# ZucksLiu/OCTCubeM

Measured on AMD Instinct MI355X. Metric: 3D-MAE pretrain volumes/s (ViT-L, 60x256x256, mask 0.75), higher is better.
Workload: dtype bf16; 1 GPU; OCTCube ViT-L 3D-MAE pre-train step (fwd+bwd+all-reduce+AdamW), synthetic (1,60,256,256) volumes, mask_ratio 0.75, decoder 512x8x16; global_batch=256, micro_batch_per_gpu=128, accum_steps=2, parallelism=dp1

## Files before the change

### octcubem_amd/csrc/attn_bwd1w.hip

```cpp
#include "attn_bwd1w.hpp"
#include "attn_bwd_tail1.hpp"
#ifndef BWD1W_TAIL_DEPTH
#define BWD1W_TAIL_DEPTH 4
#endif
#include "../../include/octmae.h"

namespace octmae {

namespace bwd1w {

constexpr int HD = 32, NW = 4, KW = 128, NG = 4, KB = NW * KW;
constexpr int LA = 3;
constexpr int NB = LA + 1;
constexpr int NOLD = 3;
using T = Tile<HD>;
constexpr int QR = 0;
constexpr int OR_ = QR + NB * T::BYTES;
constexpr int CR = OR_ + NB * T::BYTES;
constexpr int IMG = CR + NB * 512;
constexpr int IMG_BUF = KB * 64;
constexpr int OLD = IMG + 2 * IMG_BUF;
constexpr int LDS = OLD + NOLD * 2 * NW * 1024;
constexpr int STG = IMG;
static_assert(LDS <= 160 * 1024, "LDS budget");
static_assert((CR % 128) == 0 && (IMG % 128) == 0 && (OLD % 128) == 0, "XOR chunk selectors act on address bits 0..6");

using namespace bwd1w_util;

#ifdef BWD1W_STAMP
__device__ unsigned g_bwd1w_stamp[512 * 4 * 2 * 10];
#define STAMP(k) asm volatile("s_memtime %0" : "=s"(st_[k]))
#define STAMP_ACCUM(s)                                                                                           \
  do {                                                                                                           \
    asm volatile("s_waitcnt lgkmcnt(0)" : "+s"(st_[0]), "+s"(st_[1]), "+s"(st_[2]), "+s"(st_[3]), "+s"(st_[4]), \
                 "+s"(st_[5]), "+s"(st_[6]), "+s"(st_[7]), "+s"(st_[8]), "+s"(st_[9]));                          \
    _Pragma("unroll") for (int k_ = 0; k_ < 9; ++k_) acc_[s][k_] += (unsigned)st_[k_ + 1] - (unsigned)st_[k_];  \
    acc_[s][9] += (unsigned)st_[0] - last_;                                                                      \
    last_ = (unsigned)st_[9];                                                                                    \
  } while (0)
#else
#define STAMP(k)
#define STAMP_ACCUM(s)
#endif

}

__global__ __launch_bounds__(256, 1) void attn_bwd_fused1w_kernel(const bf16_t* __restrict__ qkv, const bf16_t* __restrict__ dout,
                                                                  const float* __restrict__ rowc, float* __restrict__ dq_ws,
                                                                  bf16_t* __restrict__ dqkv, int N, int NPAD, int H, int nkb,
                                                                  float scale, int tail_key) {
  using namespace bwd1w;
  extern __shared__ __attribute__((aligned(128))) char smem[];
  const unsigned lds0 = (unsigned)(size_t)(__attribute__((address_space(3))) char*)smem;

  const int tid = threadIdx.x, lane = tid & 63;
  const int wid = __builtin_amdgcn_readfirstlane(tid >> 6);
  const int r = lane & 31, h = lane >> 5;
  const int bh = xcd_remap((int)blockIdx.x, (int)gridDim.x);
  const int b = bh / H, head = bh % H;
  const size_t rs = (size_t)3 * H * HD, os = (size_t)H * HD;
  const bf16_t* qb = qkv + (size_t)b * N * rs + (size_t)head * HD;
  const bf16_t* kb_ = qb + (size_t)H * HD;
  const bf16_t* vb_ = qb + (size_t)2 * H * HD;
  const bf16_t* dob = dout + (size_t)b * N * os + (size_t)head * HD;
  const float sc2 = scale * LOG2E;
  const bool half_drain = ((N - 1) & 63) < 32;
  const int ntiles = (N + 63) / 64;

  const bool isq = wid < 2;
  const i32x4_t rsD = isq ? make_rsrc(qb, (unsigned)(((size_t)(N - 1) * rs + HD) * 2)) : make_rsrc(dob, (unsigned)(((size_t)(N - 1) * os + HD) * 2));
  unsigned dvoff[2], dlds[2];
#pragma unroll
  for (int i = 0; i < 2; ++i) {
    const int piece = (wid & 1) * 2 + i;
    const int q = piece * 64 + lane;
    const int row = q / T::CHUNKS, c = (q % T::CHUNKS) ^ T::sw(row);
    dvoff[i] = (unsigned)(((size_t)row * (isq ? rs : os) + c * 8) * 2);
    dlds[i] = (unsigned)((isq ? QR : OR_) + piece * 1024);
  }
  const unsigned dstride = (unsigned)(64 * (isq ? rs : os) * 2);
  const i32x4_t rsC = make_rsrc(rowc + (size_t)(wid & 1) * gridDim.x * NPAD + (size_t)bh * NPAD, (unsigned)((size_t)NPAD * 4));
  auto issue = [&](int dt, int ct, int slot) {
#pragma unroll
    for (int i = 0; i < 2; ++i) {
      const unsigned m0v = (unsigned)__builtin_amdgcn_readfirstlane((int)(lds0 + dlds[i] + (unsigned)(slot * T::BYTES)));
      lds_dma16(m0v, dvoff[i] + (unsigned)dt * dstride, rsD);
    }
    const unsigned m0c = (unsigned)__builtin_amdgcn_readfirstlane((int)(lds0 + CR + slot * 512 + (wid & 1) * 256));
    lds_dma4(m0c, (unsigned)((ct * 64 + lane) * 4), rsC);
  };

  float* wsb = dq_ws + (size_t)bh * N * HD;
  const i32x4_t rsW = make_rsrc(wsb, (unsigned)((size_t)N * HD * 4));
  const __amdgpu_buffer_rsrc_t rsWs = __builtin_amdgcn_make_buffer_rsrc(
      reinterpret_cast<void*>(((unsigned long long)(unsigned)rsW[1] << 32) | (unsigned)rsW[0]), 0, rsW[2], 0x00020000);
  const int dt = wid & 1, qt = wid >> 1, g16 = lane >> 4, c16 = lane & 15;
  const unsigned wsoff = (unsigned)(((16 * qt + c16) * HD + 16 * dt + 4 * g16) * 4);
  constexpr unsigned WS_SUB = 32 * HD * 4, WS_TILE = 64 * HD * 4, DROP = 0x80000000u;
  auto oldreq = [&](int tile, int buf, unsigned base) {
#pragma unroll
    for (int u = 0; u < 2; ++u) {
      const unsigned m0o = (unsigned)__builtin_amdgcn_readfirstlane((int)(lds0 + OLD + ((buf * 2 + u) * NW + wid) * 1024));
      lds_dma16_ws(m0o, wsoff + base + (unsigned)tile * WS_TILE + (unsigned)u * WS_SUB, rsW);
    }
  };

  const int tq_ = (lane >> 2) & 3, tp_ = lane & 3, tgi = (lane >> 4) & 1;
  const unsigned a_const = opaque(lds0 + (unsigned)(CR + 16 * h));
  const unsigned a_row = opaque(lds0 + (unsigned)(QR + T::off(r, h)));
  const unsigned a_trlo = opaque(lds0 + (unsigned)(QR + T::off(4 * h + tq_, 2 * tgi + (tp_ >> 1)) + (tp_ & 1) * 8));
  const unsigned a_trhi = opaque(lds0 + (unsigned)(QR + T::off(4 * h + tq_ + 8, 2 * tgi + (tp_ >> 1)) + (tp_ & 1) * 8));
  const unsigned a_imgw = opaque(lds0 + (unsigned)(IMG + img_off(wid * KW + r, h)));
  const unsigned a_imglo = opaque(lds0 + (unsigned)(IMG + img_off(8 * g16 + tq_, 4 * qt + tp_)));
  const unsigned a_imghi = opaque(lds0 + (unsigned)(IMG + img_off(8 * g16 + tq_ + 4, 4 * qt + tp_)));
  const unsigned a_old = opaque(lds0 + (unsigned)(OLD + wid * 1024 + lane * 16));
  f32x16 zero16;
#pragma unroll
  for (int e = 0; e < 16; ++e) zero16[e] = 0.f;
  const f32x4 zero4 = {0.f, 0.f, 0.f, 0.f};

  for (int kb = 0; kb < nkb; ++kb) {
    const int key0 = kb * KB;
    const unsigned oldbase = kb > 0 ? 0u : DROP;
    issue(0, 0, 0);
    issue(1, 1, 1);
    issue(2, 2, 2);
    oldreq(0, 0, oldbase);
    {
#pragma unroll
      for (int i = 0; i < KB * 4 / 256; ++i) {
        const int c = tid + 256 * i;
        const int row = c >> 2, cc = c & 3;
        const u32x4 v = *reinterpret_cast<const u32x4*>(kb_ + (size_t)(key0 + row) * rs + 8 * cc);
        *reinterpret_cast<u32x2*>(smem + STG + img_off(row, 2 * cc)) = u32x2{v[0], v[1]};
        *reinterpret_cast<u32x2*>(smem + STG + img_off(row, 2 * cc + 1)) = u32x2{v[2], v[3]};
      }
    }
    bf16x8 kS[NG][2], vS[NG][2];
#pragma unroll
    for (int g = 0; g < NG; ++g) {
      const size_t krow = (size_t)(key0 + wid * KW + 32 * g + r) * rs;
#pragma unroll
      for (int s = 0; s < 2; ++s) {
        const u32x4 kv = *reinterpret_cast<const u32x4*>(kb_ + krow + 16 * s + 8 * h);
        const u32x4 vv = *reinterpret_cast<const u32x4*>(vb_ + krow + 16 * s + 8 * h);
        kS[g][s] = scale_frag(kv, sc2);
        vS[g][s] = __builtin_bit_cast(bf16x8, vv);
      }
    }
    f32x16 dk0 = zero16, dk1 = zero16, dk2 = zero16, dk3 = zero16, dv0 = zero16, dv1 = zero16, dv2 = zero16, dv3 = zero16;
    __syncthreads();
    bf16x8 kT[KB / 32];
#pragma unroll
    for (int ks = 0; ks < KB / 32; ++ks)
      kT[ks] = cat4(lds_tr_read(smem + STG + img_off(8 * g16 + tq_, 4 * dt + tp_) + ks * 2048),
                    lds_tr_read(smem + STG + img_off(8 * g16 + tq_ + 4, 4 * dt + tp_) + ks * 2048));
    __builtin_amdgcn_s_waitcnt(0xC07F);
    __syncthreads();

    wait_vm<0>();
    __builtin_amdgcn_s_barrier();

    f32x16 lse_a, dlt_a, lse_b = zero16, dlt_b = zero16, saA, dpA, saB, dpB;
    f32x4 dqA = zero4, dqB = zero4;
    bf16x8 qrowa0, qrowa1, orowa0, orowa1, qrowb0, qrowb1, orowb0, orowb1, qTa0, qTa1, oTa0, oTa1, qTb0, qTb1, oTb0, oTb1;
    u32x4 pf0 = {0u, 0u, 0u, 0u}, pf1 = pf0, dsf0 = pf0, dsf1 = pf0;
    {
#pragma unroll
      for (int G = 0; G < 4; ++G) {
        const f32x4 a = lds_ld<f32x4>(a_const + 32 * G);
        const f32x4 d = lds_ld<f32x4>(a_const + 256 + 32 * G);
#pragma unroll
        for (int e = 0; e < 4; ++e) { lse_a[4 * G + e] = a[e]; dlt_a[4 * G + e] = d[e]; }
      }
      qrowa0 = lds_ld<bf16x8>(a_row);
      orowa0 = lds_ld<bf16x8>(a_row + (OR_ - QR));
      qrowa1 = lds_ld<bf16x8>(a_row ^ 32u);
      orowa1 = lds_ld<bf16x8>((a_row ^ 32u) + (OR_ - QR));
      qTa0 = cat4(lds_tr_ld(a_trlo), lds_tr_ld(a_trhi));
      oTa0 = cat4(lds_tr_ld(a_trlo + (OR_ - QR)), lds_tr_ld(a_trhi + (OR_ - QR)));
      qTa1 = cat4(lds_tr_ld(a_trlo + 16 * 64), lds_tr_ld(a_trhi + 16 * 64));
      oTa1 = cat4(lds_tr_ld(a_trlo + 16 * 64 + (OR_ - QR)), lds_tr_ld(a_trhi + 16 * 64 + (OR_ - QR)));
      qTb0 = qTb1 = oTb0 = oTb1 = qrowb0 = qrowb1 = orowb0 = orowb1 = __builtin_bit_cast(bf16x8, pf0);
      saA = mfma32(qrowa0, kS[0][0], lse_a);
      dpA = mfma32(orowa0, vS[0][0], dlt_a);
      saA = mfma32(qrowa1, kS[0][1], saA);
      dpA = mfma32(orowa1, vS[0][1], dpA);
      saB = zero16; dpB = zero16;
    }

#ifdef BWD1W_STAMP
    unsigned long long st_[10];
    unsigned acc_[2][10] = {};
    unsigned last_ = 0;
    STAMP(9);
    asm volatile("s_waitcnt lgkmcnt(0)" : "+s"(st_[9]));
    last_ = (unsigned)st_[9];
#endif
#define BWD1W_TILE_SETUP                                                                                            \
  [[maybe_unused]] const int slot = t & (NB - 1), slotn = (t + 1) & (NB - 1);                                                        \
  [[maybe_unused]] const unsigned s_pc1 = (unsigned)(slot * 512 + 128), s_x1 = (unsigned)(slot * T::BYTES + 32 * T::ROWB);           \
  [[maybe_unused]] const unsigned s_pcn = (unsigned)(slotn * 512), s_xn = (unsigned)(slotn * T::BYTES);                              \
  [[maybe_unused]] const unsigned s_oldr = (unsigned)(((t + 2) % NOLD) * 2 * NW * 1024);                                             \
  [[maybe_unused]] const unsigned s_redoff0 = t > 0 ? (unsigned)(t - 1) * WS_TILE : DROP;                                            \
  [[maybe_unused]] const unsigned s_redoff1 = t > 0 ? (unsigned)(t - 1) * WS_TILE + WS_SUB : DROP;                                   \
  [[maybe_unused]] auto issue_tile = [&]() {                                                                                         \
    const int tn = t + LA;                                                                                          \
    issue(tn < ntiles ? tn : tn - ntiles, tn < ntiles ? tn : ntiles, tn & (NB - 1));                                \
    oldreq(t + 1, (t + 1) % NOLD, oldbase);                                                                         \
  };
    const unsigned o_imglo = a_imglo, o_imghi = a_imghi, o_old = a_old, o_wsoff = wsoff;
#define BWD1W_DRAIN_ADDRS \
  [[maybe_unused]] const unsigned a_imglo = opaque(o_imglo), a_imghi = opaque(o_imghi), a_old = opaque(o_old), wsoff = opaque(o_wsoff);
#ifndef BWD1W_VMWAIT_EXTRA
#define BWD1W_VMWAIT_EXTRA 1
#endif
#define BWD1W_WAIT(t_) do { if ((t_) > 1) wait_vm<7 + BWD1W_VMWAIT_EXTRA>(); else wait_vm<7>(); } while (0)
    const int nloop = half_drain ? ntiles - 1 : ntiles;
    for (int t = 0; t < nloop; ++t) {
      if (t > 0) BWD1W_WAIT(t);
      BWD1W_TILE_SETUP
#include "attn_bwd1w_body.inc"
    }
    if (half_drain) {
      {
        const int t = ntiles - 1;
        BWD1W_WAIT(t);
        BWD1W_TILE_SETUP
#define BWD1W_ONLY_SUBSTEP0
#include "attn_bwd1w_body.inc"
#undef BWD1W_ONLY_SUBSTEP0
      {
        BWD1W_DRAIN_ADDRS
#define BWD1W_DRAIN_SLIM1
#include "attn_bwd1w_drain.inc"
#undef BWD1W_DRAIN_SLIM1
      }
      }
      {
        const int t = ntiles;
        BWD1W_WAIT(t);
        BWD1W_TILE_SETUP
        BWD1W_DRAIN_ADDRS
#define BWD1W_DRAIN_TINY0
#include "attn_bwd1w_drain.inc"
#undef BWD1W_DRAIN_TINY0
      }
    } else {
      const int t = ntiles;
      BWD1W_WAIT(t);
      BWD1W_TILE_SETUP
      BWD1W_DRAIN_ADDRS
#define BWD1W_DRAIN_SLIM0
#include "attn_bwd1w_drain.inc"
#undef BWD1W_DRAIN_SLIM0
#define BWD1W_DRAIN_TINY1
#include "attn_bwd1w_drain.inc"
#undef BWD1W_DRAIN_TINY1
    }
#undef BWD1W_TILE_SETUP
#undef BWD1W_DRAIN_ADDRS
#ifdef BWD1W_STAMP
    if (kb == 1 && lane == 0 && blockIdx.x < 512)
      for (int s_ = 0; s_ < 2; ++s_)
        for (int k_ = 0; k_ < 10; ++k_) g_bwd1w_stamp[((blockIdx.x * 4 + wid) * 2 + s_) * 10 + k_] = acc_[s_][k_];
#endif
    asm volatile("s_nop 15\n\ts_nop 15" : "+a"(dk0), "+a"(dk1), "+a"(dk2), "+a"(dk3), "+a"(dv0), "+a"(dv1), "+a"(dv2), "+a"(dv3));
    {
      const f32x16* dks[4] = {&dk0, &dk1, &dk2, &dk3};
      const f32x16* dvs[4] = {&dv0, &dv1, &dv2, &dv3};
#pragma unroll
      for (int g = 0; g < NG; ++g) {
        bf16_t* drow = dqkv + ((size_t)b * N + key0 + wid * KW + 32 * g + r) * rs + (size_t)head * HD;
        const f32x16& dkg = *dks[g];
        const f32x16& dvg = *dvs[g];
#pragma unroll
        for (int G = 0; G < 4; ++G) {
          const u32x2 wk = {pack2bf(dkg[4 * G] * scale, dkg[4 * G + 1] * scale), pack2bf(dkg[4 * G + 2] * scale, dkg[4 * G + 3] * scale)};
          const u32x2 wv = {pack2bf(dvg[4 * G], dvg[4 * G + 1]), pack2bf(dvg[4 * G + 2], dvg[4 * G + 3])};
          *reinterpret_cast<u32x2*>(drow + (size_t)H * HD + 8 * G + 4 * h) = wk;
          *reinterpret_cast<u32x2*>(drow + (size_t)2 * H * HD + 8 * G + 4 * h) = wv;
        }
      }
    }
  }
  wait_vm<0>();
  if (tail_key >= 0) {
    __syncthreads();
    const int lane_t = lane_id_fresh();
    attn_bwd_tail1_body<HD, BWD1W_TAIL_DEPTH>(qkv, dout, rowc, dq_ws, dqkv, N, NPAD, H, tail_key, 1, scale, bh, (int)gridDim.x, reinterpret_cast<float*>(smem),
                               wid * 64 + lane_t);
  }
}

}

using namespace octmae;

#ifdef BWD1W_STAMP
extern "C" int octmae_debug_bwd1w_stamps(void* host, int nbytes) {
  return (int)hipMemcpyFromSymbol(host, HIP_SYMBOL(octmae::bwd1w::g_bwd1w_stamp), (size_t)nbytes);
}
#endif

namespace octmae {
int launch_attn_bwd_fused1w(const bf16_t* qkv, const bf16_t* dout, const float* rowc, float* dq_ws, bf16_t* dqkv, int B, int N, int NPAD,
                            int H, int nkb, float scale, int tail_key, hipStream_t st) {
  static DynLdsOnce once;
  if (int rc = once.ensure(reinterpret_cast<const void*>(attn_bwd_fused1w_kernel), bwd1w::LDS)) return rc;
  hipLaunchKernelGGL(attn_bwd_fused1w_kernel, dim3(B * H), dim3(256), bwd1w::LDS, st, qkv, dout, rowc, dq_ws, dqkv, N, NPAD, H, nkb, scale, tail_key);
  OCTMAE_LAUNCH_CHECK();
  return 0;
}
}
```

### octcubem_amd/csrc/attn_bwd1w.hpp

```cpp
#pragma once
#include "attn_tile.hpp"

namespace octmae {
namespace bwd1w_util {

typedef __attribute__((ext_vector_type(4))) float f32x4_t;
__device__ __forceinline__ f32x4 mfma16(bf16x8 a, bf16x8 b, f32x4 c) { return mfma16x16(a, b, c); }

template <int CNT>
__device__ __forceinline__ void wait_vm() {
  static_assert(CNT >= 0 && CNT < 64, "vmcnt is 6 bits");
  __builtin_amdgcn_s_waitcnt((CNT & 15) | ((CNT >> 4) << 14) | (7 << 4) | (15 << 8));
}
__device__ __forceinline__ void lds_dma16(unsigned m0v, unsigned voff, i32x4_t rsrc) {
  asm volatile("s_mov_b32 m0, %0\n\tbuffer_load_dwordx4 %1, %2, 0 offen lds" ::"s"(m0v), "v"(voff), "s"(rsrc) : "memory", "m0");
}
#ifndef BWD1W_WS_ST_AUX
#define BWD1W_WS_ST_AUX 0
#endif
#ifdef BWD1W_ST_SMALL
#define BWD1W_RVO(x) ((x) & 0xFFFFu)
#else
#define BWD1W_RVO(x) (x)
#endif
__device__ __forceinline__ void lds_dma16_ws(unsigned m0v, unsigned voff, i32x4_t rsrc) {
#ifdef BWD1W_WS_LD_NT
  asm volatile("s_mov_b32 m0, %0\n\tbuffer_load_dwordx4 %1, %2, 0 offen nt lds" ::"s"(m0v), "v"(voff), "s"(rsrc) : "memory", "m0");
#else
  asm volatile("s_mov_b32 m0, %0\n\tbuffer_load_dwordx4 %1, %2, 0 offen lds" ::"s"(m0v), "v"(voff), "s"(rsrc) : "memory", "m0");
#endif
}
__device__ __forceinline__ void lds_dma4(unsigned m0v, unsigned voff, i32x4_t rsrc) {
  asm volatile("s_mov_b32 m0, %0\n\tbuffer_load_dword %1, %2, 0 offen lds" ::"s"(m0v), "v"(voff), "s"(rsrc) : "memory", "m0");
}
__device__ __forceinline__ i32x4_t make_rsrc(const void* base, unsigned bytes) {
  const unsigned long long a = (unsigned long long)base;
  i32x4_t r = {(int)(unsigned)a, (int)(unsigned)(a >> 32), (int)bytes, 0x00020000};
  r[0] = __builtin_amdgcn_readfirstlane(r[0]);
  r[1] = __builtin_amdgcn_readfirstlane(r[1]);
  r[2] = __builtin_amdgcn_readfirstlane(r[2]);
  r[3] = __builtin_amdgcn_readfirstlane(r[3]);
  return r;
}
__device__ __forceinline__ int img_off(int row, int c8) { return row * 64 + ((c8 ^ ((row >> 1) & 7)) << 3); }

#define MFMA_ACC(acc, a, b) asm volatile(OCTMAE_MFMA32_ASM " %0, %1, %2, %0" : "+a"(acc) : "v"(a), "v"(b))
__device__ __forceinline__ int lane_id_fresh() {
  int x;
  asm volatile("v_mbcnt_lo_u32_b32 %0, -1, 0\n\tv_mbcnt_hi_u32_b32 %0, -1, %0" : "=v"(x));
  return x;
}
#ifdef ABL_NO_BARRIER
#define SUBSTEP_END(N) __builtin_amdgcn_s_waitcnt(0xC07F | 0)
#else
#define SUBSTEP_END(N)                                            \
  do {                                                            \
    __builtin_amdgcn_s_waitcnt(0xC07F | ((N) << 8));              \
    __builtin_amdgcn_s_barrier();                                 \
  } while (0)
#endif

}
}
```

### octcubem_amd/csrc/attn_bwd1w64.hip

```cpp
#include "attn_bwd1w.hpp"
#include "attn_bwd_tail1.hpp"
#ifndef BWD1W_TAIL_DEPTH
#define BWD1W_TAIL_DEPTH 4
#endif
#include "../../include/octmae.h"

namespace octmae {

namespace bwd1w64 {

constexpr int HD = 64, NW = 4, KW = 64, NG = 2, KB = NW * KW;
constexpr int LA = 3;
constexpr int NB = LA + 1;
constexpr int NOLD = 3;
using T = Tile<HD>;
constexpr int QR = 0;
constexpr int OR_ = QR + NB * T::BYTES;
constexpr int CR = OR_ + NB * T::BYTES;
constexpr int IMG = CR + NB * 512;
constexpr int IMG_BUF = KB * 64;
constexpr int OLD = IMG + 2 * IMG_BUF;
constexpr int OLD_TILE = 2 * 2 * NW * 1024;
constexpr int LDS = OLD + NOLD * OLD_TILE;
constexpr int STG = IMG;
static_assert(KB * HD * 2 <= 2 * IMG_BUF, "K staging must fit the two images");
static_assert(LDS <= 160 * 1024, "LDS budget");
static_assert((CR % 128) == 0 && (IMG % 128) == 0 && (OLD % 128) == 0, "XOR chunk selectors act on address bits 0..6");
static_assert((OR_ - QR) % 128 == 0 && T::BYTES % 128 == 0, "slot / region offsets leave the low 7 address bits alone");

using namespace bwd1w_util;

__device__ __forceinline__ int kst_off(int row, int c) {
  const int sw = (row & 1) | (((row >> 2) & 1) << 1) | (((row >> 1) & 1) << 2) | (((row >> 3) & 1) << 3);
  return row * 128 + ((c ^ sw) << 3);
}

#ifdef BWD1W_STAMP
__device__ unsigned g_bwd1w64_stamp[512 * 4 * 2 * 8];
#define STAMP(k) asm volatile("s_memtime %0" : "=s"(st_[k]))
#define STAMP_ACCUM(s)                                                                                                         \
  do {                                                                                                                         \
    asm volatile("s_waitcnt lgkmcnt(0)" : "+s"(st_[0]), "+s"(st_[1]), "+s"(st_[2]), "+s"(st_[3]), "+s"(st_[4]), "+s"(st_[5])); \
    _Pragma("unroll") for (int k_ = 0; k_ < 5; ++k_) acc_[s][k_] += (unsigned)st_[k_ + 1] - (unsigned)st_[k_];                \
    acc_[s][5] += (unsigned)st_[0] - last_;                                                                                    \
    last_ = (unsigned)st_[5];                                                                                                  \
  } while (0)
#else
#define STAMP(k)
#define STAMP_ACCUM(s)
#endif

}

__global__ __launch_bounds__(256, 1) void attn_bwd_fused1w64_kernel(const bf16_t* __restrict__ qkv, const bf16_t* __restrict__ dout,
                                                                    const float* __restrict__ rowc, float* __restrict__ dq_ws,
                                                                    bf16_t* __restrict__ dqkv, int N, int NPAD, int H, int nkb,
                                                                    float scale, int tail_key) {
  using namespace bwd1w64;
  extern __shared__ __attribute__((aligned(128))) char smem[];
  const unsigned lds0 = (unsigned)(size_t)(__attribute__((address_space(3))) char*)smem;

  const int tid = threadIdx.x, lane = tid & 63;
  const int wid = __builtin_amdgcn_readfirstlane(tid >> 6);
  const int r = lane & 31, h = lane >> 5;
  const int bh = xcd_remap((int)blockIdx.x, (int)gridDim.x);
  const int b = bh / H, head = bh % H;
  const size_t rs = (size_t)3 * H * HD, os = (size_t)H * HD;
  const bf16_t* qb = qkv + (size_t)b * N * rs + (size_t)head * HD;
  const bf16_t* kb_ = qb + (size_t)H * HD;
  const bf16_t* vb_ = qb + (size_t)2 * H * HD;
  const bf16_t* dob = dout + (size_t)b * N * os + (size_t)head * HD;
  const float sc2 = scale * LOG2E;
  const bool half_drain = ((N - 1) & 63) < 32;
  const int ntiles = (N + 63) / 64;

  const bool isq = wid < 2;
  const i32x4_t rsD = isq ? make_rsrc(qb, (unsigned)(((size_t)(N - 1) * rs + HD) * 2)) : make_rsrc(dob, (unsigned)(((size_t)(N - 1) * os + HD) * 2));
  unsigned dvoff[4], dlds[4];
#pragma unroll
  for (int i = 0; i < 4; ++i) {
    const int piece = (wid & 1) * 4 + i;
    const int q = piece * 64 + lane;
    const int row = q / T::CHUNKS, c = (q % T::CHUNKS) ^ T::sw(row);
    dvoff[i] = (unsigned)(((size_t)row * (isq ? rs : os) + c * 8) * 2);
    dlds[i] = (unsigned)((isq ? QR : OR_) + piece * 1024);
  }
  const unsigned dstride = (unsigned)(64 * (isq ? rs : os) * 2);
  const i32x4_t rsC = make_rsrc(rowc + (size_t)(wid & 1) * gridDim.x * NPAD + (size_t)bh * NPAD, (unsigned)((size_t)NPAD * 4));
  auto issue = [&](int dt, int ct, int slot) {
#pragma unroll
    for (int i = 0; i < 4; ++i) {
      const unsigned m0v = (unsigned)__builtin_amdgcn_readfirstlane((int)(lds0 + dlds[i] + (unsigned)(slot * T::BYTES)));
      lds_dma16(m0v, dvoff[i] + (unsigned)dt * dstride, rsD);
    }
    const unsigned m0c = (unsigned)__builtin_amdgcn_readfirstlane((int)(lds0 + CR + slot * 512 + (wid & 1) * 256));
    lds_dma4(m0c, (unsigned)((ct * 64 + lane) * 4), rsC);
  };

  float* wsb = dq_ws + (size_t)bh * N * HD;
  const i32x4_t rsW = make_rsrc(wsb, (unsigned)((size_t)N * HD * 4));
  const __amdgpu_buffer_rsrc_t rsWs = __builtin_amdgcn_make_buffer_rsrc(
      reinterpret_cast<void*>(((unsigned long long)(unsigned)rsW[1] << 32) | (unsigned)rsW[0]), 0, rsW[2], 0x00020000);
  const int g16 = lane >> 4, c16 = lane & 15;
#ifdef ABL_TILED_WS
  const unsigned wsoff = (unsigned)(wid * 1024 + lane * 16);
#else
  const unsigned wsoff = (unsigned)((c16 * HD + 16 * wid + 4 * g16) * 4);
#endif
  constexpr unsigned WS_QT = 16 * HD * 4, WS_SUB = 32 * HD * 4, WS_TILE = 64 * HD * 4, DROP = 0x80000000u;
  static_assert(WS_QT == 4096, "the generated body stores the second query tile at + 4096");
  auto oldreq = [&](int tile, int buf, unsigned base) {
#pragma unroll
    for (int u = 0; u < 4; ++u) {
      const unsigned m0o = (unsigned)__builtin_amdgcn_readfirstlane((int)(lds0 + OLD + buf * OLD_TILE + (u * NW + wid) * 1024));
      lds_dma16_ws(m0o, wsoff + base + (unsigned)tile * WS_TILE + (unsigned)(u >> 1) * WS_SUB + (unsigned)(u & 1) * WS_QT, rsW);
    }
  };

  const int tq_ = (lane >> 2) & 3, tp_ = lane & 3, tgi = (lane >> 4) & 1;
  const unsigned a_const = opaque(lds0 + (unsigned)(CR + 16 * h));
  const unsigned a_row = opaque(lds0 + (unsigned)(QR + T::off(r, h)));
  const unsigned a_trlo = opaque(lds0 + (unsigned)(QR + T::off(4 * h + tq_, 2 * tgi + (tp_ >> 1)) + (tp_ & 1) * 8));
  const unsigned a_trhi = opaque(lds0 + (unsigned)(QR + T::off(4 * h + tq_ + 8, 2 * tgi + (tp_ >> 1)) + (tp_ & 1) * 8));
  const unsigned a_imgw = opaque(lds0 + (unsigned)(IMG + img_off(wid * KW + r, h)));
  const unsigned a_imglo = opaque(lds0 + (unsigned)(IMG + img_off(8 * g16 + tq_, tp_)));
  const unsigned a_imghi = opaque(lds0 + (unsigned)(IMG + img_off(8 * g16 + tq_ + 4, tp_)));
  const unsigned a_old = opaque(lds0 + (unsigned)(OLD + wid * 1024 + lane * 16));
  f32x16 zero16;
#pragma unroll
  for (int e = 0; e < 16; ++e) zero16[e] = 0.f;
  const f32x4 zero4 = {0.f, 0.f, 0.f, 0.f};

#ifdef BWD1W_STAMP
  unsigned long long k0_, r0_;
  asm volatile("s_memtime %0\n\ts_memrealtime %1\n\ts_waitcnt lgkmcnt(0)" : "=s"(k0_), "=s"(r0_));
#endif
  for (int kb = 0; kb < nkb; ++kb) {
    const int key0 = kb * KB;
    const unsigned oldbase = kb > 0 ? 0u : DROP;
    issue(0, 0, 0);
    issue(1, 1, 1);
    issue(2, 2, 2);
    oldreq(0, 0, oldbase);
    {
#pragma unroll
      for (int i = 0; i < KB * 8 / 256; ++i) {
        const int c = tid + 256 * i;
        const int row = c >> 3, cc = c & 7;
        const u32x4 v = *reinterpret_cast<const u32x4*>(kb_ + (size_t)(key0 + row) * rs + 8 * cc);
        *reinterpret_cast<u32x2*>(smem + STG + kst_off(row, 2 * cc)) = u32x2{v[0], v[1]};
        *reinterpret_cast<u32x2*>(smem + STG + kst_off(row, 2 * cc + 1)) = u32x2{v[2], v[3]};
      }
    }
    bf16x8 kS[NG][4], vS[NG][4];
#pragma unroll
    for (int g = 0; g < NG; ++g) {
      const size_t krow = (size_t)(key0 + wid * KW + 32 * g + r) * rs;
#pragma unroll
      for (int s = 0; s < 4; ++s) {
        const u32x4 kv = *reinterpret_cast<const u32x4*>(kb_ + krow + 16 * s + 8 * h);
        const u32x4 vv = *reinterpret_cast<const u32x4*>(vb_ + krow + 16 * s + 8 * h);
        kS[g][s] = scale_frag(kv, sc2);
        vS[g][s] = __builtin_bit_cast(bf16x8, vv);
      }
    }
    f32x16 dk00 = zero16, dk01 = zero16, dk10 = zero16, dk11 = zero16, dv00 = zero16, dv01 = zero16, dv10 = zero16, dv11 = zero16;
    __syncthreads();
    bf16x8 kT[KB / 32];
#pragma unroll
    for (int ks = 0; ks < KB / 32; ++ks)
      kT[ks] = cat4(lds_tr_read(smem + STG + kst_off(8 * g16 + tq_, 4 * wid + tp_) + ks * 32 * 128),
                    lds_tr_read(smem + STG + kst_off(8 * g16 + tq_ + 4, 4 * wid + tp_) + ks * 32 * 128));
    __builtin_amdgcn_s_waitcnt(0xC07F);
    __syncthreads();

    wait_vm<0>();
    __builtin_amdgcn_s_barrier();

    f32x16 lse_t, dlt_t, saA, dpA, saB = zero16, dpB = zero16;
    f32x4 dqA0 = zero4, dqA1 = zero4, dqB0 = zero4, dqB1 = zero4;
    bf16x8 qrow0, qrow1, qrow2, qrow3, orow0, orow1, orow2, orow3, qT0d0, qT0d1, oT0d0, oT0d1, qT1d0, qT1d1, oT1d0, oT1d1;
    u32x4 pf0 = {0u, 0u, 0u, 0u}, pf1 = pf0, dsf0 = pf0, dsf1 = pf0;
    {
#pragma unroll
      for (int G = 0; G < 4; ++G) {
        const f32x4 a = lds_ld<f32x4>(a_const + 32 * G);
        const f32x4 d = lds_ld<f32x4>(a_const + 256 + 32 * G);
#pragma unroll
        for (int e = 0; e < 4; ++e) { lse_t[4 * G + e] = a[e]; dlt_t[4 * G + e] = d[e]; }
      }
      qrow0 = lds_ld<bf16x8>(a_row);
      orow0 = lds_ld<bf16x8>(a_row + (OR_ - QR));
      qrow1 = lds_ld<bf16x8>(a_row ^ 32u);
      orow1 = lds_ld<bf16x8>((a_row ^ 32u) + (OR_ - QR));
      qrow2 = lds_ld<bf16x8>(a_row ^ 64u);
      orow2 = lds_ld<bf16x8>((a_row ^ 64u) + (OR_ - QR));
      qrow3 = lds_ld<bf16x8>(a_row ^ 96u);
      orow3 = lds_ld<bf16x8>((a_row ^ 96u) + (OR_ - QR));
      qT0d0 = cat4(lds_tr_ld(a_trlo), lds_tr_ld(a_trhi));
      oT0d0 = cat4(lds_tr_ld(a_trlo + (OR_ - QR)), lds_tr_ld(a_trhi + (OR_ - QR)));
      qT0d1 = cat4(lds_tr_ld(a_trlo ^ 64u), lds_tr_ld(a_trhi ^ 64u));
      oT0d1 = cat4(lds_tr_ld((a_trlo ^ 64u) + (OR_ - QR)), lds_tr_ld((a_trhi ^ 64u) + (OR_ - QR)));
      qT1d0 = qT1d1 = oT1d0 = oT1d1 = __builtin_bit_cast(bf16x8, pf0);
      saA = mfma32(qrow0, kS[0][0], lse_t);
      dpA = mfma32(orow0, vS[0][0], dlt_t);
      saA = mfma32(qrow1, kS[0][1], saA);
      dpA = mfma32(orow1, vS[0][1], dpA);
      saA = mfma32(qrow2, kS[0][2], saA);
      dpA = mfma32(orow2, vS[0][2], dpA);
      saA = mfma32(qrow3, kS[0][3], saA);
      dpA = mfma32(orow3, vS[0][3], dpA);
    }

#ifdef BWD1W_STAMP
    unsigned long long st_[6], sw_[2];
    unsigned acc_[2][8] = {};
    unsigned last_ = 0;
    STAMP(5);
    asm volatile("s_waitcnt lgkmcnt(0)" : "+s"(st_[5]));
    last_ = (unsigned)st_[5];
#endif
#define BWD1W_TILE_SETUP                                                                                                        \
  [[maybe_unused]] const int slot = t & (NB - 1), slotn = (t + 1) & (NB - 1);                                                                    \
  [[maybe_unused]] const unsigned s_x0 = (unsigned)(slot * T::BYTES), s_x1 = s_x0 + 32 * T::ROWB, s_xn = (unsigned)(slotn * T::BYTES);           \
  [[maybe_unused]] const unsigned s_pc1 = (unsigned)(slot * 512 + 128), s_pcn = (unsigned)(slotn * 512);                                         \
  [[maybe_unused]] const unsigned s_oldr = (unsigned)(((t + 2) % NOLD) * OLD_TILE);                                                              \
  [[maybe_unused]] const unsigned s_redoff0 = t > 0 ? (unsigned)(t - 1) * WS_TILE : DROP;                                                        \
  [[maybe_unused]] const unsigned s_redoff1 = t > 0 ? (unsigned)(t - 1) * WS_TILE + WS_SUB : DROP;                                               \
  [[maybe_unused]] auto issue_tile = [&]() {                                                                                                     \
    const int tn = t + LA;                                                                                                      \
    issue(BWD1W_DMA_TILE(tn), tn < ntiles ? tn : ntiles, tn & (NB - 1));                                                        \
    oldreq(t + 1, (t + 1) % NOLD, BWD1W_OLD_BASE);                                                                              \
  };
#ifdef ABL_NO_TILE_DMA
#define BWD1W_DMA_TILE(tn) 0
#else
#define BWD1W_DMA_TILE(tn) ((tn) < ntiles ? (tn) : (tn) - ntiles)
#endif
#ifdef ABL_NO_OLDREQ
#define BWD1W_OLD_BASE DROP
#else
#define BWD1W_OLD_BASE oldbase
#endif
    const unsigned o_imglo = a_imglo, o_imghi = a_imghi, o_old = a_old, o_wsoff = wsoff;
#define BWD1W_DRAIN_ADDRS \
  [[maybe_unused]] const unsigned a_imglo = opaque(o_imglo), a_imghi = opaque(o_imghi), a_old = opaque(o_old), wsoff = opaque(o_wsoff);
#ifndef BWD1W_VMWAIT_EXTRA
#define BWD1W_VMWAIT_EXTRA 2
#endif
#define BWD1W_WAIT(t_) do { if ((t_) > 1) wait_vm<13 + BWD1W_VMWAIT_EXTRA>(); else wait_vm<13>(); } while (0)
    const int nloop = half_drain ? ntiles - 1 : ntiles + 1;
    for (int t = 0; t < nloop; ++t) {
#ifdef BWD1W_STAMP
      asm volatile("s_memtime %0\n\ts_waitcnt lgkmcnt(0)" : "=s"(sw_[0]));
#endif
      if (t > 0) BWD1W_WAIT(t);
#ifdef BWD1W_STAMP
      asm volatile("s_memtime %0\n\ts_waitcnt lgkmcnt(0)" : "=s"(sw_[1]));
      acc_[0][6] += (unsigned)sw_[1] - (unsigned)sw_[0];
#endif
      BWD1W_TILE_SETUP
#include "attn_bwd1w_body_hd64.inc"
    }
    if (half_drain) {
      {
        const int t = ntiles - 1;
        BWD1W_WAIT(t);
        BWD1W_TILE_SETUP
#define BWD1W_ONLY_SUBSTEP0
#include "attn_bwd1w_body_hd64.inc"
#undef BWD1W_ONLY_SUBSTEP0
      {
        BWD1W_DRAIN_ADDRS
#define BWD1W_DRAIN_SLIM1
#include "attn_bwd1w_drain_hd64.inc"
#undef BWD1W_DRAIN_SLIM1
      }
      }
      {
        const int t = ntiles;
        BWD1W_WAIT(t);
        BWD1W_TILE_SETUP
        BWD1W_DRAIN_ADDRS
#define BWD1W_DRAIN_TINY0
#include "attn_bwd1w_drain_hd64.inc"
#undef BWD1W_DRAIN_TINY0
      }
    }
#undef BWD1W_TILE_SETUP
#undef BWD1W_DRAIN_ADDRS
#ifdef BWD1W_STAMP
    if (kb == 1 && lane == 0 && blockIdx.x < 512)
      for (int s_ = 0; s_ < 2; ++s_)
        for (int k_ = 0; k_ < 8; ++k_) g_bwd1w64_stamp[((blockIdx.x * 4 + wid) * 2 + s_) * 8 + k_] = acc_[s_][k_];
#endif
    asm volatile("s_nop 15\n\ts_nop 15" : "+a"(dk00), "+a"(dk01), "+a"(dk10), "+a"(dk11), "+a"(dv00), "+a"(dv01), "+a"(dv10), "+a"(dv11));
#ifdef ABL_NO_EPI
    if (N < 0)
#endif
    {
      const f32x16* dks[2][2] = {{&dk00, &dk01}, {&dk10, &dk11}};
      const f32x16* dvs[2][2] = {{&dv00, &dv01}, {&dv10, &dv11}};
      const int le = (int)opaque((unsigned)lane);
      const int re = le & 31, he = le >> 5;
      char* stg = smem + IMG + wid * (KW * 128);
      bf16_t* dbase = dqkv + ((size_t)b * N + key0 + wid * KW) * rs + (size_t)head * HD;
#pragma unroll
      for (int which = 0; which < 2; ++which) {
#pragma unroll
        for (int g = 0; g < NG; ++g)
#pragma unroll
          for (int d = 0; d < 2; ++d) {
            const f32x16& acc = which ? *dvs[g][d] : *dks[g][d];
            const float sc = which ? 1.0f : scale;
            const int row = 32 * g + re;
#pragma unroll
            for (int G = 0; G < 4; ++G) {
              const u32x2 w = {pack2bf(acc[4 * G] * sc, acc[4 * G + 1] * sc), pack2bf(acc[4 * G + 2] * sc, acc[4 * G + 3] * sc)};
              *reinterpret_cast<u32x2*>(stg + row * 128 + (((8 * d + 2 * G + he) ^ (row & 15)) << 3)) = w;
            }
          }
#pragma unroll
        for (int i = 0; i < KW / 8; ++i) {
          const int row = 8 * i + (le >> 3), j = le & 7, x = row & 15;
          const u32x4 v = *reinterpret_cast<const u32x4*>(stg + row * 128 + ((j ^ (x >> 1)) << 4));
          const u32x4 o = (x & 1) ? u32x4{v[2], v[3], v[0], v[1]} : v;
          *reinterpret_cast<u32x4*>(dbase + (size_t)row * rs + (size_t)(1 + which) * H * HD + 8 * j) = o;
        }
      }
    }
    __builtin_amdgcn_s_waitcnt(0xC07F);
    __builtin_amdgcn_s_barrier();
  }
  wait_vm<0>();
  if (tail_key >= 0) {
    __syncthreads();
    const int lane_t = lane_id_fresh();
    attn_bwd_tail1_body<HD, BWD1W_TAIL_DEPTH>(qkv, dout, rowc, dq_ws, dqkv, N, NPAD, H, tail_key, 1, scale, bh, (int)gridDim.x, reinterpret_cast<float*>(smem),
                               wid * 64 + lane_t);
  }
#ifdef BWD1W_STAMP
  {
    unsigned long long k1_, r1_;
    asm volatile("s_memtime %0\n\ts_memrealtime %1\n\ts_waitcnt lgkmcnt(0)" : "=s"(k1_), "=s"(r1_));
    if (lane == 0 && blockIdx.x < 512) {
      g_bwd1w64_stamp[((blockIdx.x * 4 + wid) * 2 + 0) * 8 + 7] = (unsigned)(k1_ - k0_);
      g_bwd1w64_stamp[((blockIdx.x * 4 + wid) * 2 + 1) * 8 + 7] = (unsigned)(r1_ - r0_);
    }
  }
#endif
}

}
#ifdef BWD1W_STAMP
extern "C" int octmae_debug_bwd1w64_stamps(void* host, int nbytes) {
  return (int)hipMemcpyFromSymbol(host, HIP_SYMBOL(octmae::bwd1w64::g_bwd1w64_stamp), (size_t)nbytes);
}
#endif
namespace octmae {

int launch_attn_bwd_fused1w64(const bf16_t* qkv, const bf16_t* dout, const float* rowc, float* dq_ws, bf16_t* dqkv, int B, int N, int NPAD,
                              int H, int nkb, float scale, int tail_key, hipStream_t st) {
  static DynLdsOnce once;
  if (int rc = once.ensure(reinterpret_cast<const void*>(attn_bwd_fused1w64_kernel), bwd1w64::LDS)) return rc;
  hipLaunchKernelGGL(attn_bwd_fused1w64_kernel, dim3(B * H), dim3(256), bwd1w64::LDS, st, qkv, dout, rowc, dq_ws, dqkv, N, NPAD, H, nkb, scale, tail_key);
  OCTMAE_LAUNCH_CHECK();
  return 0;
}

}
```

Before: 166.1 volumes/s.

## Prefetch next key/value block into registers during attention backward drain

In the head-dim-64 fused attention backward kernel, global loads of the next key block (staging data and V fragments) and the LDS DMA requests now go out at the end of the current block, before the dK/dV epilogue, rather than at the start of the next iteration. K fragments are now read back from the swizzled LDS staging area instead of being loaded a second time from global memory. Optional compile-time phase timers are added to both kernels. The goal is to hide global load latency behind the epilogue and to cut redundant K reads. The cost is more live registers for the prefetch buffers in a launch-bounds-1 kernel and an extra barrier per block.

```diff
diff --git a/octcubem_amd/csrc/attn_bwd1w.hip b/octcubem_amd/csrc/attn_bwd1w.hip
--- a/octcubem_amd/csrc/attn_bwd1w.hip
+++ b/octcubem_amd/csrc/attn_bwd1w.hip
@@ -43,6 +43,15 @@
 #define STAMP_ACCUM(s)
 #endif
 
+#ifdef BWD1W_PHASES
+__device__ unsigned g_bwd1w_phase[512 * 4 * 16];
+#define PHASE_MARK() asm volatile("s_memrealtime %0\n\ts_waitcnt lgkmcnt(0)" : "=s"(pl_))
+#define PHASE(i) do { unsigned long long n_; asm volatile("s_memrealtime %0\n\ts_waitcnt lgkmcnt(0)" : "=s"(n_)); pd_[i] = (unsigned)(n_ - pl_); pl_ = n_; } while (0)
+#else
+#define PHASE_MARK()
+#define PHASE(i)
+#endif
+
 }
 
 __global__ __launch_bounds__(256, 1) void attn_bwd_fused1w_kernel(const bf16_t* __restrict__ qkv, const bf16_t* __restrict__ dout,
@@ -119,9 +128,15 @@
   for (int e = 0; e < 16; ++e) zero16[e] = 0.f;
   const f32x4 zero4 = {0.f, 0.f, 0.f, 0.f};
 
+#ifdef BWD1W_PHASES
+  unsigned long long p0_, pl_;
+  asm volatile("s_memrealtime %0\n\ts_waitcnt lgkmcnt(0)" : "=s"(p0_));
+  unsigned pd_[8] = {};
+#endif
   for (int kb = 0; kb < nkb; ++kb) {
     const int key0 = kb * KB;
     const unsigned oldbase = kb > 0 ? 0u : DROP;
+    PHASE_MARK();
     issue(0, 0, 0);
     issue(1, 1, 1);
     issue(2, 2, 2);
@@ -150,6 +165,7 @@
     }
     f32x16 dk0 = zero16, dk1 = zero16, dk2 = zero16, dk3 = zero16, dv0 = zero16, dv1 = zero16, dv2 = zero16, dv3 = zero16;
     __syncthreads();
+    PHASE(0);
     bf16x8 kT[KB / 32];
 #pragma unroll
     for (int ks = 0; ks < KB / 32; ++ks)
@@ -157,9 +173,11 @@
                     lds_tr_read(smem + STG + img_off(8 * g16 + tq_ + 4, 4 * dt + tp_) + ks * 2048));
     __builtin_amdgcn_s_waitcnt(0xC07F);
     __syncthreads();
+    PHASE(1);
 
     wait_vm<0>();
     __builtin_amdgcn_s_barrier();
+    PHASE(2);
 
     f32x16 lse_a, dlt_a, lse_b = zero16, dlt_b = zero16, saA, dpA, saB, dpB;
     f32x4 dqA = zero4, dqB = zero4;
@@ -189,6 +207,7 @@
       saB = zero16; dpB = zero16;
     }
 
+    PHASE(3);
 #ifdef BWD1W_STAMP
     unsigned long long st_[10];
     unsigned acc_[2][10] = {};
@@ -222,6 +241,7 @@
       BWD1W_TILE_SETUP
 #include "attn_bwd1w_body.inc"
     }
+    PHASE(4);
     if (half_drain) {
       {
         const int t = ntiles - 1;
@@ -260,6 +280,7 @@
     }
 #undef BWD1W_TILE_SETUP
 #undef BWD1W_DRAIN_ADDRS
+    PHASE(5);
 #ifdef BWD1W_STAMP
     if (kb == 1 && lane == 0 && blockIdx.x < 512)
       for (int s_ = 0; s_ < 2; ++s_)
@@ -283,14 +304,30 @@
         }
       }
     }
+#ifdef BWD1W_PHASES
+    PHASE(6);
+    if (kb == 1 && lane == 0 && blockIdx.x < 512)
+      for (int k_ = 0; k_ < 7; ++k_) g_bwd1w_phase[(blockIdx.x * 4 + wid) * 16 + k_] = pd_[k_];
+#endif
   }
   wait_vm<0>();
+  PHASE_MARK();
   if (tail_key >= 0) {
     __syncthreads();
     const int lane_t = lane_id_fresh();
     attn_bwd_tail1_body<HD, BWD1W_TAIL_DEPTH>(qkv, dout, rowc, dq_ws, dqkv, N, NPAD, H, tail_key, 1, scale, bh, (int)gridDim.x, reinterpret_cast<float*>(smem),
                                wid * 64 + lane_t);
   }
+#ifdef BWD1W_PHASES
+  {
+    unsigned long long p1_;
+    asm volatile("s_memrealtime %0\n\ts_waitcnt lgkmcnt(0)" : "=s"(p1_));
+    if (lane == 0 && blockIdx.x < 512) {
+      g_bwd1w_phase[(blockIdx.x * 4 + wid) * 16 + 7] = (unsigned)(p1_ - pl_);
+      g_bwd1w_phase[(blockIdx.x * 4 + wid) * 16 + 8] = (unsigned)(p1_ - p0_);
+    }
+  }
+#endif
 }
 
 }
@@ -313,3 +350,9 @@
   return 0;
 }
 }
+
+#ifdef BWD1W_PHASES
+extern "C" int octmae_debug_bwd1w_phases(void* host, int nbytes) {
+  return (int)hipMemcpyFromSymbol(host, HIP_SYMBOL(octmae::bwd1w::g_bwd1w_phase), (size_t)nbytes);
+}
+#endif
diff --git a/octcubem_amd/csrc/attn_bwd1w.hpp b/octcubem_amd/csrc/attn_bwd1w.hpp
--- a/octcubem_amd/csrc/attn_bwd1w.hpp
+++ b/octcubem_amd/csrc/attn_bwd1w.hpp
@@ -45,6 +45,10 @@
 __device__ __forceinline__ int img_off(int row, int c8) { return row * 64 + ((c8 ^ ((row >> 1) & 7)) << 3); }
 
 #define MFMA_ACC(acc, a, b) asm volatile(OCTMAE_MFMA32_ASM " %0, %1, %2, %0" : "+a"(acc) : "v"(a), "v"(b))
+__device__ __forceinline__ int opaque_s(int v) {
+  asm volatile("" : "+s"(v));
+  return v;
+}
 __device__ __forceinline__ int lane_id_fresh() {
   int x;
   asm volatile("v_mbcnt_lo_u32_b32 %0, -1, 0\n\tv_mbcnt_hi_u32_b32 %0, -1, %0" : "=v"(x));
diff --git a/octcubem_amd/csrc/attn_bwd1w64.hip b/octcubem_amd/csrc/attn_bwd1w64.hip
--- a/octcubem_amd/csrc/attn_bwd1w64.hip
+++ b/octcubem_amd/csrc/attn_bwd1w64.hip
@@ -50,6 +50,15 @@
 #define STAMP_ACCUM(s)
 #endif
 
+#ifdef BWD1W_PHASES
+__device__ unsigned g_bwd1w64_phase[512 * 4 * 16];
+#define PHASE_MARK() asm volatile("s_memrealtime %0\n\ts_waitcnt lgkmcnt(0)" : "=s"(pl_))
+#define PHASE(i) do { unsigned long long n_; asm volatile("s_memrealtime %0\n\ts_waitcnt lgkmcnt(0)" : "=s"(n_)); pd_[i] = (unsigned)(n_ - pl_); pl_ = n_; } while (0)
+#else
+#define PHASE_MARK()
+#define PHASE(i)
+#endif
+
 }
 
 __global__ __launch_bounds__(256, 1) void attn_bwd_fused1w64_kernel(const bf16_t* __restrict__ qkv, const bf16_t* __restrict__ dout,
@@ -135,47 +144,86 @@
   unsigned long long k0_, r0_;
   asm volatile("s_memtime %0\n\ts_memrealtime %1\n\ts_waitcnt lgkmcnt(0)" : "=s"(k0_), "=s"(r0_));
 #endif
+#ifdef BWD1W_PHASES
+  unsigned long long p0_, pl_;
+  asm volatile("s_memrealtime %0\n\ts_waitcnt lgkmcnt(0)" : "=s"(p0_));
+  unsigned pd_[8] = {};
+#endif
+  u32x4 kst[KB * 8 / 256], vraw[NG][4];
+  auto request_block = [&](int key0, unsigned oldbase) {
+    const int one = opaque_s(1);
+    issue(0, 0, 0);
+    issue(one, one, 1);
+    issue(2 * one, 2 * one, 2);
+    oldreq(0, 0, oldbase);
+    const int te = wid * 64 + lane_id_fresh();
+#pragma unroll
+    for (int i = 0; i < KB * 8 / 256; ++i) {
+      const int c = te + 256 * i;
+      kst[i] = *reinterpret_cast<const u32x4*>(kb_ + (size_t)(key0 + (c >> 3)) * rs + 8 * (c & 7));
+    }
+    const int rf = te & 31, hf = (te >> 5) & 1;
+#pragma unroll
+    for (int g = 0; g < NG; ++g) {
+      const size_t krow = (size_t)(key0 + wid * KW + 32 * g + rf) * rs;
+#pragma unroll
+      for (int s = 0; s < 4; ++s)
+        vraw[g][s] = *reinterpret_cast<const u32x4*>(vb_ + krow + 16 * s + 8 * hf);
+    }
+  };
+  if (nkb > 0) request_block(0, DROP);
   for (int kb = 0; kb < nkb; ++kb) {
     const int key0 = kb * KB;
     const unsigned oldbase = kb > 0 ? 0u : DROP;
-    issue(0, 0, 0);
-    issue(1, 1, 1);
-    issue(2, 2, 2);
-    oldreq(0, 0, oldbase);
+    PHASE_MARK();
     {
+      const int tf = wid * 64 + lane_id_fresh();
 #pragma unroll
       for (int i = 0; i < KB * 8 / 256; ++i) {
-        const int c = tid + 256 * i;
+        const int c = tf + 256 * i;
         const int row = c >> 3, cc = c & 7;
-        const u32x4 v = *reinterpret_cast<const u32x4*>(kb_ + (size_t)(key0 + row) * rs + 8 * cc);
+        const u32x4 v = kst[i];
         *reinterpret_cast<u32x2*>(smem + STG + kst_off(row, 2 * cc)) = u32x2{v[0], v[1]};
         *reinterpret_cast<u32x2*>(smem + STG + kst_off(row, 2 * cc + 1)) = u32x2{v[2], v[3]};
       }
     }
     bf16x8 kS[NG][4], vS[NG][4];
 #pragma unroll
-    for (int g = 0; g < NG; ++g) {
-      const size_t krow = (size_t)(key0 + wid * KW + 32 * g + r) * rs;
-#pragma unroll
-      for (int s = 0; s < 4; ++s) {
-        const u32x4 kv = *reinterpret_cast<const u32x4*>(kb_ + krow + 16 * s + 8 * h);
-        const u32x4 vv = *reinterpret_cast<const u32x4*>(vb_ + krow + 16 * s + 8 * h);
-        kS[g][s] = scale_frag(kv, sc2);
-        vS[g][s] = __builtin_bit_cast(bf16x8, vv);
-      }
-    }
+    for (int g = 0; g < NG; ++g)
+#pragma unroll
+      for (int s = 0; s < 4; ++s) vS[g][s] = __builtin_bit_cast(bf16x8, vraw[g][s]);
     f32x16 dk00 = zero16, dk01 = zero16, dk10 = zero16, dk11 = zero16, dv00 = zero16, dv01 = zero16, dv10 = zero16, dv11 = zero16;
     __syncthreads();
+    PHASE(0);
+    {
+      const int lf = lane_id_fresh();
+      const int rf = lf & 31, hf = lf >> 5;
+#pragma unroll
+      for (int g = 0; g < NG; ++g) {
+        const int row = wid * KW + 32 * g + rf;
+#pragma unroll
+        for (int s = 0; s < 4; ++s) {
+          const u32x4 v = *reinterpret_cast<const u32x4*>(smem + STG + (kst_off(row, 4 * s + 2 * hf) & ~15));
+          const u32x4 kv = (row & 1) ? u32x4{v[2], v[3], v[0], v[1]} : v;
+          kS[g][s] = scale_frag(kv, sc2);
+        }
+      }
+    }
     bf16x8 kT[KB / 32];
-#pragma unroll
-    for (int ks = 0; ks < KB / 32; ++ks)
-      kT[ks] = cat4(lds_tr_read(smem + STG + kst_off(8 * g16 + tq_, 4 * wid + tp_) + ks * 32 * 128),
-                    lds_tr_read(smem + STG + kst_off(8 * g16 + tq_ + 4, 4 * wid + tp_) + ks * 32 * 128));
+    {
+      const int lk = lane_id_fresh();
+      const int krow = 8 * (lk >> 4) + ((lk >> 2) & 3), kc = 4 * wid + (lk & 3);
+#pragma unroll
+      for (int ks = 0; ks < KB / 32; ++ks)
+        kT[ks] = cat4(lds_tr_read(smem + STG + kst_off(krow, kc) + ks * 32 * 128), lds_tr_read(smem + STG + kst_off(krow + 4, kc) + ks * 32 * 128));
+    }
     __builtin_amdgcn_s_waitcnt(0xC07F);
     __syncthreads();
+    PHASE(1);
 
     wait_vm<0>();
     __builtin_amdgcn_s_barrier();
+    PHASE(2);
 
     f32x16 lse_t, dlt_t, saA, dpA, saB = zero16, dpB = zero16;
     f32x4 dqA0 = zero4, dqA1 = zero4, dqB0 = zero4, dqB1 = zero4;
@@ -212,6 +260,7 @@
       dpA = mfma32(orow3, vS[0][3], dpA);
     }
 
+    PHASE(3);
 #ifdef BWD1W_STAMP
     unsigned long long st_[6], sw_[2];
     unsigned acc_[2][8] = {};
@@ -262,9 +311,10 @@
       BWD1W_TILE_SETUP
 #include "attn_bwd1w_body_hd64.inc"
     }
+    PHASE(4);
     if (half_drain) {
       {
-        const int t = ntiles - 1;
+        const int t = opaque_s(ntiles - 1);
         BWD1W_WAIT(t);
         BWD1W_TILE_SETUP
 #define BWD1W_ONLY_SUBSTEP0
@@ -278,7 +328,7 @@
       }
       }
       {
-        const int t = ntiles;
+        const int t = opaque_s(ntiles);
         BWD1W_WAIT(t);
         BWD1W_TILE_SETUP
         BWD1W_DRAIN_ADDRS
@@ -289,11 +339,17 @@
     }
 #undef BWD1W_TILE_SETUP
 #undef BWD1W_DRAIN_ADDRS
+    PHASE(5);
 #ifdef BWD1W_STAMP
     if (kb == 1 && lane == 0 && blockIdx.x < 512)
       for (int s_ = 0; s_ < 2; ++s_)
         for (int k_ = 0; k_ < 8; ++k_) g_bwd1w64_stamp[((blockIdx.x * 4 + wid) * 2 + s_) * 8 + k_] = acc_[s_][k_];
 #endif
+    if (kb + 1 < nkb) {
+      __builtin_amdgcn_s_waitcnt(0xC07F);
+      __builtin_amdgcn_s_barrier();
+      request_block(key0 + KB, 0u);
+    }
     asm volatile("s_nop 15\n\ts_nop 15" : "+a"(dk00), "+a"(dk01), "+a"(dk10), "+a"(dk11), "+a"(dv00), "+a"(dv01), "+a"(dv10), "+a"(dv11));
 #ifdef ABL_NO_EPI
     if (N < 0)
@@ -301,7 +357,7 @@
     {
       const f32x16* dks[2][2] = {{&dk00, &dk01}, {&dk10, &dk11}};
       const f32x16* dvs[2][2] = {{&dv00, &dv01}, {&dv10, &dv11}};
-      const int le = (int)opaque((unsigned)lane);
+      const int le = lane_id_fresh();
       const int re = le & 31, he = le >> 5;
       char* stg = smem + IMG + wid * (KW * 128);
       bf16_t* dbase = dqkv + ((size_t)b * N + key0 + wid * KW) * rs + (size_t)head * HD;
@@ -331,8 +387,14 @@
     }
     __builtin_amdgcn_s_waitcnt(0xC07F);
     __builtin_amdgcn_s_barrier();
+#ifdef BWD1W_PHASES
+    PHASE(6);
+    if (kb == 1 && lane == 0 && blockIdx.x < 512)
+      for (int k_ = 0; k_ < 7; ++k_) g_bwd1w64_phase[(blockIdx.x * 4 + wid) * 16 + k_] = pd_[k_];
+#endif
   }
   wait_vm<0>();
+  PHASE_MARK();
   if (tail_key >= 0) {
     __syncthreads();
     const int lane_t = lane_id_fresh();
@@ -349,12 +411,27 @@
     }
   }
 #endif
+#ifdef BWD1W_PHASES
+  {
+    unsigned long long p1_;
+    asm volatile("s_memrealtime %0\n\ts_waitcnt lgkmcnt(0)" : "=s"(p1_));
+    if (lane == 0 && blockIdx.x < 512) {
+      g_bwd1w64_phase[(blockIdx.x * 4 + wid) * 16 + 7] = (unsigned)(p1_ - pl_);
+      g_bwd1w64_phase[(blockIdx.x * 4 + wid) * 16 + 8] = (unsigned)(p1_ - p0_);
+    }
+  }
+#endif
 }
 
 }
 #ifdef BWD1W_STAMP
 extern "C" int octmae_debug_bwd1w64_stamps(void* host, int nbytes) {
   return (int)hipMemcpyFromSymbol(host, HIP_SYMBOL(octmae::bwd1w64::g_bwd1w64_stamp), (size_t)nbytes);
+}
+#endif
+#ifdef BWD1W_PHASES
+extern "C" int octmae_debug_bwd1w64_phases(void* host, int nbytes) {
+  return (int)hipMemcpyFromSymbol(host, HIP_SYMBOL(octmae::bwd1w64::g_bwd1w64_phase), (size_t)nbytes);
 }
 #endif
 namespace octmae {
```

New measurement: 166.2 volumes/s (median of 3 runs). About the same (+0.0%).
